# kofinandi/pixel-nerf-yolo

Measured on AMD Instinct MI355X. Metric: rays/sec (whole node), 64 samples/ray, 3-view 128×128 render, higher is better.
Workload: dtype f32 (matrix products on f16x2 split operands, fp32 accumulate)

## Files before the change

pixel-nerf-yolo_amd/csrc/mlp_h2.hip:

```cpp
#include <cstdlib>
#include <cstring>
#include <cstdio>
#include <vector>

#include "mlp_bwd_core.h"
#include "mlp_h2_core.h"

#if PNY_H2_PLANES == 1
#define PNY_H2_KERNEL pny_mlp_h1_kernel
#elif defined(PNY_H2_SPLIT)
#define PNY_H2_KERNEL pny_mlp_h2s_kernel
#else
#define PNY_H2_KERNEL pny_mlp_h2_kernel
#endif

namespace pny {

#ifdef PNY_H2_STAMP
enum { HS_TOTAL = 0, HS_GEMM, HS_GATHER_WAIT, HS_GATHER, HS_EPI_WAIT, HS_EPI, HS_PROLOGUE, HS_LINOUT, HS_SLAB, HS_REAL, HS_N };
__device__ unsigned long long* g_h2_stamp_buf;
__device__ __forceinline__ unsigned long long h2now() {
    unsigned long long t;
    __builtin_amdgcn_sched_barrier(0);
    asm volatile("s_memtime %0\n\ts_waitcnt lgkmcnt(0)" : "=s"(t)::"memory");
    __builtin_amdgcn_sched_barrier(0);
    return t;
}
#define HS_T0() hs_t_ = h2now()
#define HS_LAP(cat)                         \
    {                                       \
        const unsigned long long n_ = h2now(); \
        hs_acc[cat] += n_ - hs_t_;          \
        hs_t_ = n_;                         \
    }
#else
#define HS_T0()
#define HS_LAP(cat)
#endif


__device__ __forceinline__ void stash_store(__amdgpu_buffer_rsrc_t rsrc, unsigned voff, unsigned soff, float a, float b, float c, float d) {
    const f32x4 v = {a, b, c, d};
    __builtin_amdgcn_raw_buffer_store_b128(__builtin_bit_cast(u32x4, v), rsrc, voff + soff, 0, 0);
}

template <bool SIGNED = false>
__device__ __forceinline__ void h2put_planes(char* slot, float r0, float r1, float r2, float r3, float& rmax) {
    if constexpr (SIGNED)
        rmax = fmaxf(fmaxf(rmax, fmaxf(fabsf(r0), fabsf(r1))), fmaxf(fabsf(r2), fabsf(r3)));
    else
        rmax = fmaxf(fmaxf(rmax, fmaxf(r0, r1)), fmaxf(r2, r3));
    put_planes(slot, r0, r1, r2, r3);
}
__device__ __forceinline__ void range_check(float rmax, unsigned* range_flag) {
    if (__builtin_expect(!(rmax < 65520.0f), 0)) range_report(range_flag, 1u);
}

template <bool ADDZ, bool STASH = false>
__device__ __forceinline__ void h2epilogue(f32x16 (&acc)[h2::NT][h2::MT], const float* bias, char* planes, int wave, int lane, unsigned* range_flag,
                                           __amdgpu_buffer_rsrc_t stash = __amdgpu_buffer_rsrc_t(), unsigned stash_off = 0) {
    using namespace h2;
    const unsigned stash_lane = (unsigned)(((8 * NT * wave + (lane >> 5)) * TM + (lane & 31)) * 16);
    const int m0 = lane & 31, hh = lane >> 5;
    const float* bl = bias + 32 * NT * wave + 4 * hh;
    float rmax = 0.f;
    char* base = planes + (4 * NT * wave) * (2 * ROW_BYTES) + m0 * 16 + 8 * hh;
#pragma unroll
    for (int nt = 0; nt < NT; ++nt) {
        float4 b[4];
#pragma unroll
        for (int q = 0; q < 4; ++q) b[q] = *reinterpret_cast<const float4*>(bl + 32 * nt + 8 * q);
#pragma unroll
        for (int mt = 0; mt < MT; ++mt) {
            float2 za[4], zb[4];
            if (ADDZ) {
#pragma unroll
                for (int q = 0; q < 4; ++q) {
                    const char* s0 = base + (4 * nt + q) * (2 * ROW_BYTES) + 32 * mt * 16;
                    za[q] = *reinterpret_cast<const float2*>(s0);
                    zb[q] = *reinterpret_cast<const float2*>(s0 + ROW_BYTES);
                }
            }
            __builtin_amdgcn_sched_barrier(0);
#pragma unroll
            for (int q = 0; q < 4; ++q) {
                char* s0 = base + (4 * nt + q) * (2 * ROW_BYTES) + 32 * mt * 16;
                float x0 = acc[nt][mt][4 * q + 0] + b[q].x, x1 = acc[nt][mt][4 * q + 1] + b[q].y;
                float x2 = acc[nt][mt][4 * q + 2] + b[q].z, x3 = acc[nt][mt][4 * q + 3] + b[q].w;
                if (ADDZ) {
                    x0 += za[q].x;
                    x1 += za[q].y;
                    x2 += zb[q].x;
                    x3 += zb[q].y;
                }
                acc[nt][mt][4 * q + 0] = x0;
                acc[nt][mt][4 * q + 1] = x1;
                acc[nt][mt][4 * q + 2] = x2;
                acc[nt][mt][4 * q + 3] = x3;
                const float r0 = relu1(x0), r1 = relu1(x1), r2 = relu1(x2), r3 = relu1(x3);
                if constexpr (STASH) stash_store(stash, stash_lane, stash_off + (unsigned)(((8 * nt + 2 * q) * TM + 32 * mt) * 16), r0, r1, r2, r3);
                h2put_planes(s0, r0, r1, r2, r3, rmax);
            }
        }
    }
    range_check(rmax, range_flag);
}

struct SlabRef {
    __amdgpu_buffer_rsrc_t rsrc;
    unsigned lane_off;
};
__device__ __forceinline__ void h2slab_store(const f32x16 (&h)[h2::NT][h2::MT], const SlabRef& sl) {
    using namespace h2;
#pragma unroll
    for (int nt = 0; nt < NT; ++nt)
#pragma unroll
        for (int mt = 0; mt < MT; ++mt)
#pragma unroll
            for (int q = 0; q < 4; ++q) {
// ... 4 lines not shown
}
__device__ __forceinline__ void h2slab_load(f32x16 (&t)[h2::NT][h2::MT], const SlabRef& sl) {
    using namespace h2;
#pragma unroll
    for (int nt = 0; nt < NT; ++nt)
#pragma unroll
        for (int mt = 0; mt < MT; ++mt)
#pragma unroll
            for (int q = 0; q < 4; ++q) {
                const u32x4 u = __builtin_amdgcn_raw_buffer_load_b128(sl.rsrc, sl.lane_off, (unsigned)(((nt * MT + mt) * 4 + q) * 64 * 16), 2);
                const f32x4 v = __builtin_bit_cast(f32x4, u);
                t[nt][mt][4 * q + 0] = v.x;
                t[nt][mt][4 * q + 1] = v.y;
                t[nt][mt][4 * q + 2] = v.z;
                t[nt][mt][4 * q + 3] = v.w;
            }
}

#ifndef PNY_H2_SLAB_DEPTH
#define PNY_H2_SLAB_DEPTH 4
#endif
struct SlabPipe {
    static constexpr int SD = PNY_H2_SLAB_DEPTH;
    static_assert(SD >= 2, "slab pipeline");
    f32x4 buf[SD][4];
};
__device__ __forceinline__ void h2slab_issue(SlabPipe& sp, int p, const SlabRef& sh, const SlabRef& sr) {
    const SlabRef& s = (p & 1) ? sh : sr;
#pragma unroll
    for (int q = 0; q < 4; ++q)
        sp.buf[p % SlabPipe::SD][q] =
            __builtin_bit_cast(f32x4, __builtin_amdgcn_raw_buffer_load_b128(s.rsrc, s.lane_off, (unsigned)(((p >> 1) * 4 + q) * 64 * 16), 2));
}
__device__ __forceinline__ void h2view_sum(f32x16 (&net)[h2::NT][h2::MT], f32x16 (&h)[h2::NT][h2::MT], const float* bias, const SlabRef& sh,
                                           const SlabRef& sr, bool add, bool store, int wave, int lane) {
    using namespace h2;
    SlabPipe sp;
    const float* bl = bias + 32 * NT * wave + 4 * (lane >> 5);
    constexpr int NP = 2 * NT * MT, SD = SlabPipe::SD;
    if (add) {
#pragma unroll
        for (int p = 0; p + 1 < SD; ++p) h2slab_issue(sp, p, sh, sr);
    }
#pragma unroll
    for (int p = 0; p < NP; ++p) {
        const int nt = (p >> 1) / MT, mt = (p >> 1) % MT;
        if (add) {
            if (p + SD - 1 < NP) h2slab_issue(sp, p + SD - 1, sh, sr);
            __builtin_amdgcn_sched_barrier(0);
        }
        f32x16& t = (p & 1) ? h[nt][mt] : net[nt][mt];
#pragma unroll
        for (int q = 0; q < 4; ++q) {
            if (!(p & 1)) {
                const float4 b = *reinterpret_cast<const float4*>(bl + 32 * nt + 8 * q);
                t[4 * q + 0] = relu1(t[4 * q + 0] + b.x);
                t[4 * q + 1] = relu1(t[4 * q + 1] + b.y);
                t[4 * q + 2] = relu1(t[4 * q + 2] + b.z);
                t[4 * q + 3] = relu1(t[4 * q + 3] + b.w);
            }
            if (add) {
#pragma unroll
                for (int i = 0; i < 4; ++i) t[4 * q + i] = t[4 * q + i] + sp.buf[p % SD][q][i];
            }
            if (store) {
                const SlabRef& s = (p & 1) ? sh : sr;
                const f32x4 v = {t[4 * q + 0], t[4 * q + 1], t[4 * q + 2], t[4 * q + 3]};
                __builtin_amdgcn_raw_buffer_store_b128(__builtin_bit_cast(u32x4, v), s.rsrc, s.lane_off + (unsigned)(((p >> 1) * 4 + q) * 64 * 16), 0, 2);
            }
        }
        if (add) __builtin_amdgcn_sched_barrier(0);
    }
}

__device__ __forceinline__ void h2mean_planes(const f32x16 (&net)[h2::NT][h2::MT], f32x16 (&h)[h2::NT][h2::MT], float rns, char* planes, int wave,
                                              int lane, unsigned* range_flag) {
    using namespace h2;
    float rmax = 0.f;
    char* base = planes + (4 * NT * wave) * (2 * ROW_BYTES) + (lane & 31) * 16 + 8 * (lane >> 5);
#pragma unroll
    for (int nt = 0; nt < NT; ++nt)
#pragma unroll
        for (int mt = 0; mt < MT; ++mt)
#pragma unroll
            for (int q = 0; q < 4; ++q) {
                char* s0 = base + (4 * nt + q) * (2 * ROW_BYTES) + 32 * mt * 16;
                const float r0 = net[nt][mt][4 * q + 0] * rns, r1 = net[nt][mt][4 * q + 1] * rns;
                const float r2 = net[nt][mt][4 * q + 2] * rns, r3 = net[nt][mt][4 * q + 3] * rns;
                h2put_planes(s0, r0, r1, r2, r3, rmax);
#pragma unroll
                for (int i = 0; i < 4; ++i) h[nt][mt][4 * q + i] = h[nt][mt][4 * q + i] * rns;
            }
    range_check(rmax, range_flag);
}

template <int B>
__device__ __forceinline__ void h2gather_commit(const GatherTaps<h2::C, 2>& g, char* planes, int chunk, int wave, int lane) {
    using namespace h2;
    constexpr int NMB = GatherTaps<C>::NMB, QSTEP = GatherTaps<C>::QSTEP;
    const int m = (wave % NMB) * 8 + (lane & 7);
    char* base = planes + (16 * chunk + (lane >> 4)) * (2 * ROW_BYTES) + m * 16 + 8 * ((lane >> 3) & 1);
#pragma unroll
    for (int i = 0; i < GatherTaps<C>::QPW; ++i) {
        const int qb = wave / NMB + i * QSTEP;
        const float4 r = tap_blend(g.x[B][i], g.w);
        char* s0 = base + (4 * qb) * (2 * ROW_BYTES);
        *reinterpret_cast<float2*>(s0) = make_float2(r.x, r.y);
        *reinterpret_cast<float2*>(s0 + ROW_BYTES) = make_float2(r.z, r.w);
    }
}

struct WaveGather {
    f32x4 x[2][4][4];
};
template <int B, int T>
__device__ __forceinline__ void h2wave_issue(WaveGather& wg, __amdgpu_buffer_rsrc_t zr, const float4* tap_tab, unsigned c0, int lane) {
    using namespace h2;
    constexpr int nt = T / MT, mt = T % MT;
    asm volatile("" : "+v"(lane));
    const float4* tt = tap_tab + 2 * (32 * mt + (lane >> 3));
    const unsigned ql = 16u * (unsigned)(lane & 7);
#pragma unroll
    for (int pass = 0; pass < 4; ++pass) {
        const float4 o = tt[16 * pass];
        const unsigned off[4] = {(unsigned)__float_as_int(o.x), (unsigned)__float_as_int(o.y), (unsigned)__float_as_int(o.z), (unsigned)__float_as_int(o.w)};
#pragma unroll
        for (int k = 0; k < 4; ++k)
            wg.x[B][pass][k] = __builtin_bit_cast(f32x4, __builtin_amdgcn_raw_buffer_load_b128(zr, off[k] * 4u + ql, c0 + 128u * nt, 0));
    }
}
template <int B, int T>
__device__ __forceinline__ void h2wave_commit(const WaveGather& wg, f32x16 (&acc)[h2::NT][h2::MT], const float4* tap_tab, const float* bias,
                                              char* planes, int wave, int lane, float& rmax) {
    using namespace h2;
    constexpr int nt = T / MT, mt = T % MT;
    const int jq = lane & 7, sl = lane >> 3, m0 = lane & 31, hh = lane >> 5;
    char* tb = planes + (4 * NT * wave + 4 * nt) * (2 * ROW_BYTES) + 32 * mt * 16;
    char* wr = tb + jq * ROW_BYTES + 16 * (sl ^ jq);
    const float4* tw = tap_tab + 2 * (32 * mt + sl) + 1;
#pragma unroll
    for (int pass = 0; pass < 4; ++pass) {
        const float4 w4 = tw[16 * pass];
        const float w[4] = {w4.x, w4.y, w4.z, w4.w};
        float4 x[4];
#pragma unroll
        for (int k = 0; k < 4; ++k) x[k] = make_float4(wg.x[B][pass][k][0], wg.x[B][pass][k][1], wg.x[B][pass][k][2], wg.x[B][pass][k][3]);
        *reinterpret_cast<float4*>(wr + 128 * pass) = tap_blend(x, w);
    }
    __builtin_amdgcn_fence(__ATOMIC_RELEASE, "wavefront");
    __builtin_amdgcn_wave_barrier();
    __builtin_amdgcn_fence(__ATOMIC_ACQUIRE, "wavefront");
    const float* bl = bias + 32 * NT * wave + 32 * nt + 4 * hh;
    auto rd_b = [&](int q) { return *reinterpret_cast<const float4*>(bl + 8 * q); };
    auto rd_z = [&](int q) { return *reinterpret_cast<const float4*>(tb + (2 * q + hh) * ROW_BYTES + 16 * (m0 ^ (2 * q + hh))); };
    float4 b = rd_b(0), z = rd_z(0);
#pragma unroll
    for (int q = 0; q < 4; ++q) {
        const float4 bq = b, zq = z;
        if (q + 1 < 4) b = rd_b(q + 1), z = rd_z(q + 1);
        __builtin_amdgcn_fence(__ATOMIC_ACQ_REL, "wavefront");
        char* s0 = tb + q * (2 * ROW_BYTES) + m0 * 16 + 8 * hh;
        float x0 = acc[nt][mt][4 * q + 0] + bq.x, x1 = acc[nt][mt][4 * q + 1] + bq.y;
        float x2 = acc[nt][mt][4 * q + 2] + bq.z, x3 = acc[nt][mt][4 * q + 3] + bq.w;
        x0 += zq.x;
        x1 += zq.y;
        x2 += zq.z;
        x3 += zq.w;
        acc[nt][mt][4 * q + 0] = x0;
        acc[nt][mt][4 * q + 1] = x1;
        acc[nt][mt][4 * q + 2] = x2;
        acc[nt][mt][4 * q + 3] = x3;
        const float r0 = relu1(x0), r1 = relu1(x1), r2 = relu1(x2), r3 = relu1(x3);
        h2put_planes(s0, r0, r1, r2, r3, rmax);
    }
}
__device__ __forceinline__ void h2wave_entry(WaveGather& wg, f32x16 (&acc)[h2::NT][h2::MT], __amdgpu_buffer_rsrc_t zr, const float4* tap_tab, unsigned c0,
                                             const float* bias, char* planes, int wave, int lane, unsigned* range_flag) {
    static_assert(h2::NT * h2::MT == 4, "four sub-chunks");
    asm volatile("" : "+v"(lane));
    float rmax = 0.f;
    h2wave_issue<1, 1>(wg, zr, tap_tab, c0, lane);
    __builtin_amdgcn_sched_barrier(0);
    h2wave_commit<0, 0>(wg, acc, tap_tab, bias, planes, wave, lane, rmax);
    h2wave_issue<0, 2>(wg, zr, tap_tab, c0, lane);
    __builtin_amdgcn_sched_barrier(0);
    h2wave_commit<1, 1>(wg, acc, tap_tab, bias, planes, wave, lane, rmax);
    h2wave_issue<1, 3>(wg, zr, tap_tab, c0, lane);
    __builtin_amdgcn_sched_barrier(0);
    h2wave_commit<0, 2>(wg, acc, tap_tab, bias, planes, wave, lane, rmax);
    h2wave_commit<1, 3>(wg, acc, tap_tab, bias, planes, wave, lane, rmax);
    range_check(rmax, range_flag);
}

#if PNY_H2_PLANES == 2
struct LinOutW {
    h8 f[2 * h2::NT][2];
};
__device__ __forceinline__ void h2linout_issue(LinOutW& lw, const WStream& ws, unsigned img_off, int nto_n, int nto, int wave) {
    using namespace h2;
    unsigned base = img_off + (unsigned)(((2 * NT * wave * nto_n + nto) * 2) * 64) * 16u, step = (unsigned)(nto_n * 2 * 64) * 16u;
    asm volatile("" : "+s"(base), "+s"(step));
#pragma unroll
    for (int ks = 0; ks < 2 * NT; ++ks)
#pragma unroll
        for (int p = 0; p < 2; ++p)
            lw.f[ks][p] = __builtin_bit_cast(h8, __builtin_amdgcn_raw_buffer_load_b128(ws.rsrc, ws.lane_off, base + ks * step + (unsigned)(p * 64) * 16u, 0));
}
constexpr int LINOUT_WAVE_BYTES = 4 * h2::NT * 2 * h2::ROW_BYTES;
static_assert((h2::NT / 2) * h2::TM * 16 * 16 <= LINOUT_WAVE_BYTES, "a wave's partials (64 outputs) fit its own rows");
__device__ __forceinline__ void h2linout_product(LinOutW& lw, const WStream& ws, unsigned img_off, int d_out, char* planes, int wave, int lane) {
    using namespace h2;
    constexpr int NCH = NT / 2;
    asm volatile("" : "+v"(lane));
    const int m0 = lane & 31, hh = lane >> 5;
    const int qo = (d_out + 3) >> 2, nto_n = d_out > 32 ? 2 : 1;
    char* region = planes + wave * LINOUT_WAVE_BYTES;
    __builtin_amdgcn_fence(__ATOMIC_RELEASE, "wavefront");
    __builtin_amdgcn_wave_barrier();
    __builtin_amdgcn_fence(__ATOMIC_ACQUIRE, "wavefront");
    h8 B[NCH][MT][4][2];
#pragma unroll
    for (int c = 0; c < NCH; ++c)
#pragma unroll
// ... 42 lines not shown
    static_assert(NCHUNK * 64 == HID, "eight chunks of 64 k");
    asm volatile("" : "+v"(tid));
    const int qo = (a.d_out + 3) >> 2;
    const bool vec = a.d_out == 4 && (reinterpret_cast<size_t>(a.out) & 15) == 0;
    for (int idx = tid; idx < qo * TM; idx += THREADS) {
        const int qd = idx / TM, m = idx % TM;
        const char* src = planes + (m * qo + qd) * 16;
        f32x4 part[NCHUNK];
#pragma unroll
        for (int g = 0; g < NCHUNK; ++g) part[g] = *reinterpret_cast<const f32x4*>(src + (g / NCH) * LINOUT_WAVE_BYTES + (g % NCH) * (TM * qo * 16));
        float sum[4];
#pragma unroll
        for (int i = 0; i < 4; ++i) {
            sum[i] = part[0][i];
#pragma unroll
            for (int g = 1; g < NCHUNK; ++g) sum[i] = sum[i] + part[g][i];
        }
        const long long s = tile * TM + m;
        if (s >= a.n_points) continue;
        if (vec) {
#pragma unroll
            for (int i = 0; i < 4; ++i) sum[i] = output_head(sum[i] + a.w.b_out[i], i, a.yolo);
            *reinterpret_cast<float4*>(a.out + s * 4) = make_float4(sum[0], sum[1], sum[2], sum[3]);
        } else {
#pragma unroll
            for (int i = 0; i < 4; ++i) {
                const int o = 4 * qd + i;
                if (o < a.d_out) a.out[s * a.d_out + o] = output_head(sum[i] + a.w.b_out[o], o, a.yolo);
            }
        }
    }
}
#endif

template <bool STASH>
__device__ __forceinline__ void h2prologue(const MlpArgs& a, int v, long long tile, char* planes, float4* tap_tab, int tid, unsigned* range_flag,
                                           __amdgpu_buffer_rsrc_t stash = __amdgpu_buffer_rsrc_t(), unsigned stash_xin = 0, float4* tap_raw = nullptr) {
    using namespace h2;
    constexpr int NPART = THREADS / TM;
    const int m = tid % TM, part = tid / TM;
    long long s = tile * TM + m;
    if (s >= a.n_points) s = a.n_points - 1;
    float p[3], d[3];
    load_point(a, s, p, d);
    const Cam cam = a.cams[tile_view_base(a, tile * TM) + v];
    float xr[3], xc[3], vd[3];
    camera_point(cam, p, d, xr, xc, vd);
    float rmax = 0.f;
    for (int g = part; g < D_IN_PAD / 4; g += NPART) {
        const float e0 = input_entry(4 * g + 0, xr, vd, a.freq_factor, a.num_freqs), e1 = input_entry(4 * g + 1, xr, vd, a.freq_factor, a.num_freqs);
        const float e2 = input_entry(4 * g + 2, xr, vd, a.freq_factor, a.num_freqs), e3 = input_entry(4 * g + 3, xr, vd, a.freq_factor, a.num_freqs);
        if constexpr (STASH) stash_store(stash, (unsigned)((g * TM + m) * 16), stash_xin, e0, e1, e2, e3);
        h2put_planes<true>(planes + (g >> 1) * (2 * ROW_BYTES) + m * 16 + 8 * (g & 1), e0, e1, e2, e3, rmax);
    }
    range_check(rmax, range_flag);
    if (part == NPART - 1) {
        int pix[4], offs[4];
        float wgt[4];
        pixel_taps(a, cam, xc, 1, pix, wgt);
#pragma unroll
        for (int k = 0; k < 4; ++k) offs[k] = pix[k] * a.tap_stride;
        tap_record(tap_tab, m, offs, wgt);
        if constexpr (STASH) {
#pragma unroll
            for (int k = 0; k < 4; ++k) offs[k] = pix[k] * a.L;
            tap_record(tap_raw, m, offs, wgt);
        }
    }
}

template <bool STASH>
__global__ __launch_bounds__(h2::THREADS, 2) void PNY_H2_KERNEL(const MlpArgs a) {
    using namespace h2;
    extern __shared__ __attribute__((aligned(16))) char smem_raw[];
    char* planes = smem_raw;
    float4* tap_tab = reinterpret_cast<float4*>(smem_raw + ACT_BYTES);
    float* bias_tab = reinterpret_cast<float*>(smem_raw + ACT_BYTES + TAP_BYTES);
    float4* tap_raw = reinterpret_cast<float4*>(smem_raw + lds_bytes(a.n_blocks));
    const int tid = threadIdx.x, lane = tid & 63, wave = __builtin_amdgcn_readfirstlane(tid >> 6);
    const SlabRef slab = {__builtin_amdgcn_make_buffer_rsrc(a.scratch + (size_t)blockIdx.x * (TM * HID), 0, TM * HID * 4, 0x00020000),
                          (unsigned)((wave * (NT * MT * 16 * 64) + 4 * lane) * 4)};
#if defined(PNY_H2_PER_VIEW_FC1) || PNY_H2_PLANES == 1
    constexpr bool VIEW_MEAN = false;
#else
    constexpr bool VIEW_MEAN = !STASH;
#endif
    constexpr bool WAVE_ENTRY = !STASH;
    const SlabRef slab_r = {__builtin_amdgcn_make_buffer_rsrc(a.scratch + ((size_t)gridDim.x + blockIdx.x) * (TM * HID), 0, TM * HID * 4, 0x00020000),
                            slab.lane_off};
    const int nb = a.n_blocks;
    const int nvb = a.combine_layer < nb ? a.combine_layer : nb;
    const WStream ws = wstream(a, lane);
    const H2Seg s_in = h2seg(ws, a.h2_in, D_IN_PAD / 16, wave);
    auto fc0seg = [&](int b) { return h2seg(ws, a.h2_fc0[b], HID / 16, wave); };
    auto fc1seg = [&](int b) { return h2seg(ws, a.h2_fc1[b], HID / 16, wave); };
    auto entry_bias = [&](int b) -> const float* {
        if constexpr (LDS_BIAS) return bias_tab + (b == 0 ? 0 : 2 * b) * HID;
        return b == 0 ? a.w.b_in : a.w.b_fc1[b - 1];
    };
    auto fc0_bias = [&](int b) -> const float* {
        if constexpr (LDS_BIAS) return bias_tab + (1 + 2 * b) * HID;
        return a.w.b_fc0[b];
    };
    H2Ring ring;
    h2ring_fill(ring, ws, s_in);
#ifdef PNY_H2_STAMP
    unsigned long long hs_acc[HS_N], hs_t_ = 0;
    for (int i = 0; i < HS_N; ++i) hs_acc[i] = 0;
    const unsigned long long hs_start = h2now();
    const unsigned long long hs_real0 = __builtin_amdgcn_s_memrealtime();
#endif
    if constexpr (LDS_BIAS) {
        for (int i = tid; i < (1 + 2 * nb) * HID; i += THREADS) {
            const int vec = i / HID, f = i % HID;
            const float* src = vec == 0 ? a.w.b_in : ((vec & 1) ? a.w.b_fc0[(vec - 1) >> 1] : a.w.b_fc1[(vec - 2) >> 1]);
            bias_tab[i] = src[f];
        }
    }

    const TileWalk tw = tile_walk(a.n_tiles);
    for (long long tile = tw.first; tile < tw.last; tile += tw.step) {
        f32x16 h[NT][MT];
        f32x16 net[NT][MT];
        GatherTaps<C, 2> g;
        WaveGather wg;
        __amdgpu_buffer_rsrc_t zr = __amdgpu_buffer_rsrc_t();
        const unsigned wave_c0 = (unsigned)(32 * NT * wave) * 4u;
        auto prefetch = [&](int c0) {
            if constexpr (WAVE_ENTRY)
                h2wave_issue<0, 0>(wg, zr, tap_tab, (unsigned)c0 * 4u + wave_c0, lane);
            else
                gather_issue<C, 0>(g, c0, wave);
        };
        __amdgpu_buffer_rsrc_t xr = __amdgpu_buffer_rsrc_t();
        if constexpr (STASH)
            xr = stash_rsrc(a.lay.x_record(a.stash_x, tile), a.lay.x_tile);
        auto block_tail = [&](int blk, const H2Seg& after, bool slab_in, int next_c0, unsigned stash_net) {
            HS_T0();
            h2zero<NT, MT>(net);
            __syncthreads();
            HS_LAP(HS_EPI_WAIT);
            h2gemm(net, ring, ws, fc0seg(blk), fc1seg(blk), planes, lane);
            HS_LAP(HS_GEMM);
            __syncthreads();
            HS_LAP(HS_EPI_WAIT);
            h2epilogue<false, STASH>(net, fc0_bias(blk), planes, wave, lane, a.range_flag, xr, stash_net);
            if (!VIEW_MEAN && slab_in) {
                h2slab_load(net, slab);
                HS_LAP(HS_EPI);
                __syncthreads();
                HS_LAP(HS_EPI_WAIT);
                h2gemm(h, ring, ws, fc1seg(blk), after, planes, lane);
                HS_LAP(HS_GEMM);
#pragma unroll
                for (int nt = 0; nt < NT; ++nt)
#pragma unroll
                    for (int mt = 0; mt < MT; ++mt)
#pragma unroll
                        for (int r = 0; r < 16; ++r) h[nt][mt][r] = net[nt][mt][r] + h[nt][mt][r];
            } else if (next_c0 >= 0) {
                HS_LAP(HS_EPI);
                __syncthreads();
                HS_LAP(HS_EPI_WAIT);
                h2gemm(h, ring, ws, fc1seg(blk), after, planes, lane, [&]() { prefetch(next_c0); });
                HS_LAP(HS_GEMM);
            } else {
                HS_LAP(HS_EPI);
                __syncthreads();
                HS_LAP(HS_EPI_WAIT);
                h2gemm(h, ring, ws, fc1seg(blk), after, planes, lane);
                HS_LAP(HS_GEMM);
            }
        };
        for (int v = 0; v < a.NS; ++v) {
            const int vb = tile_view_base(a, tile * TM);
            const H2Seg after_view = v + 1 < a.NS ? s_in : (nvb < nb ? fc0seg(nvb) : s_in);
            const unsigned x_view = STASH ? stash_bytes((unsigned)v * (unsigned)a.lay.x_view) : 0u;
            auto act_slot = [&](int i) { return x_view + stash_bytes((unsigned)a.lay.o_act + (unsigned)i * (unsigned)STASH_SLOT); };
            HS_T0();
            __syncthreads();
            h2prologue<STASH>(a, v, tile, planes, tap_tab, tid, a.range_flag, xr, x_view + stash_bytes((unsigned)a.lay.o_in), tap_raw);
            h2zero<NT, MT>(h);
            __syncthreads();
            if constexpr (STASH) {
                const unsigned xz = x_view + stash_bytes((unsigned)a.lay.o_z);
                gather_setup<C>(g, a.latent + (size_t)(vb + v) * a.Hl * a.Wl * a.L, tap_raw, wave, lane);
                const int nch = a.L / GCH;
                const unsigned zlane = (unsigned)(((lane >> 3) * TM + (wave % 8) * 8 + (lane & 7)) * 16);
                auto put = [&](const float4(&x)[4][4], int c) {
#pragma unroll
                    for (int i = 0; i < 4; ++i) {
                        const float4 r = tap_blend(x[i], g.w);
                        stash_store(xr, zlane, xz + (unsigned)((32 * c + 8 * i) * TM * 16), r.x, r.y, r.z, r.w);
                    }
                };
                gather_issue<C, 0>(g, 0, wave);
                for (int c = 0; c < nch; c += 2) {
                    if (c + 1 < nch) gather_issue<C, 1>(g, (c + 1) * GCH, wave);
                    __builtin_amdgcn_sched_barrier(0);
                    put(g.x[0], c);
                    if (c + 2 < nch) gather_issue<C, 0>(g, (c + 2) * GCH, wave);
                    __builtin_amdgcn_sched_barrier(0);
                    if (c + 1 < nch) put(g.x[1], c + 1);
                }
            }
            if constexpr (WAVE_ENTRY) {
                const size_t zfloats = (size_t)a.Hl * a.Wl * a.zp_stride;
                zr = __builtin_amdgcn_make_buffer_rsrc(const_cast<float*>(a.zp) + (size_t)(vb + v) * zfloats, 0, (int)(unsigned)(zfloats * 4), 0x00020000);
            } else {
                gather_setup<C>(g, a.zp + (size_t)(vb + v) * a.Hl * a.Wl * a.zp_stride, tap_tab, wave, lane);
            }
            prefetch(0);
            HS_LAP(HS_PROLOGUE);
            h2gemm(h, ring, ws, s_in, fc0seg(0), planes, lane);
            HS_LAP(HS_GEMM);
            auto block_entry = [&](int blk) {
                const int cb = blk * HID;
                HS_LAP(HS_GATHER);
                __syncthreads();
                HS_LAP(HS_GATHER_WAIT);
                if constexpr (WAVE_ENTRY) {
                    h2wave_entry(wg, h, zr, tap_tab, (unsigned)cb * 4u + wave_c0, entry_bias(blk), planes, wave, lane, a.range_flag);
                    HS_LAP(HS_GATHER);
                    return;
                }
                gather_issue<C, 1>(g, cb + GCH, wave);
                __builtin_amdgcn_sched_barrier(0);
                h2gather_commit<0>(g, planes, 0, wave, lane);
                gather_issue<C, 0>(g, cb + 2 * GCH, wave);
                __builtin_amdgcn_sched_barrier(0);
                h2gather_commit<1>(g, planes, 1, wave, lane);
                gather_issue<C, 1>(g, cb + 3 * GCH, wave);
                __builtin_amdgcn_sched_barrier(0);
                h2gather_commit<0>(g, planes, 2, wave, lane);
                h2gather_commit<1>(g, planes, 3, wave, lane);
                HS_LAP(HS_GATHER);
                __syncthreads();
                HS_LAP(HS_GATHER_WAIT);
                h2epilogue<true, STASH>(h, entry_bias(blk), planes, wave, lane, a.range_flag, xr, act_slot(2 * blk));
                HS_LAP(HS_EPI);
            };
            auto view_block = [&](int blk, const H2Seg& after, bool slab_in, int next_c0) {
                block_entry(blk);
                block_tail(blk, after, slab_in, next_c0, act_slot(2 * blk + 1));
            };
            auto mean_tail = [&](int blk) {
                const bool last = v + 1 == a.NS;
                HS_T0();
                h2zero<NT, MT>(net);
                __syncthreads();
                HS_LAP(HS_EPI_WAIT);
                h2gemm(net, ring, ws, fc0seg(blk), last ? fc1seg(blk) : s_in, planes, lane);
                HS_LAP(HS_GEMM);
                h2view_sum(net, h, fc0_bias(blk), slab, slab_r, v > 0, !last, wave, lane);
                if (!last) {
                    HS_LAP(HS_SLAB);
                    return;
                }
                HS_LAP(v > 0 ? HS_SLAB : HS_EPI);
                __syncthreads();
                HS_LAP(HS_EPI_WAIT);
                h2mean_planes(net, h, 1.0f / (float)a.NS, planes, wave, lane, a.range_flag);
                HS_LAP(HS_EPI);
                __syncthreads();
                HS_LAP(HS_EPI_WAIT);
                h2gemm(h, ring, ws, fc1seg(blk), after_view, planes, lane);
                HS_LAP(HS_GEMM);
            };
#if defined(PNY_H2_NOPREFETCH)
            for (int blk = 0; blk + 1 < nvb; ++blk) {
                view_block(blk, fc0seg(blk + 1), false, -1);
                prefetch((blk + 1) * HID);
            }
#else
            for (int blk = 0; blk + 1 < nvb; ++blk) view_block(blk, fc0seg(blk + 1), false, (blk + 1) * HID);
#endif
            if constexpr (VIEW_MEAN) {
                block_entry(nvb - 1);
                mean_tail(nvb - 1);
            } else {
                view_block(nvb - 1, after_view, v > 0, -1);
            }
            if (!VIEW_MEAN && a.NS > 1) {
                HS_T0();
                if (v + 1 < a.NS) {
                    h2slab_store(h, slab);
                } else {
                    const float rns = 1.0f / (float)a.NS;
#pragma unroll
                    for (int nt = 0; nt < NT; ++nt)
#pragma unroll
                        for (int mt = 0; mt < MT; ++mt)
#pragma unroll
                            for (int r = 0; r < 16; ++r) h[nt][mt][r] = h[nt][mt][r] * rns;
                }
                HS_LAP(HS_SLAB);
            }
        }
        auto post_slot = [&](int i) { return stash_bytes((unsigned)a.lay.x_post + (unsigned)i * (unsigned)STASH_SLOT); };
        for (int blk = nvb; blk < nb; ++blk) {
            HS_T0();
            __syncthreads();
            HS_LAP(HS_EPI_WAIT);
            h2epilogue<false, STASH>(h, entry_bias(blk), planes, wave, lane, a.range_flag, xr, post_slot(2 * (blk - nvb)));
            HS_LAP(HS_EPI);
            block_tail(blk, blk + 1 < nb ? fc0seg(blk + 1) : s_in, false, -1, post_slot(2 * (blk - nvb) + 1));
        }
        HS_T0();
#if PNY_H2_PLANES == 2
        const unsigned out_off = (unsigned)(reinterpret_cast<const char*>(a.h2_out) - ws.base);
        LinOutW lw;
        h2linout_issue(lw, ws, out_off, a.d_out > 32 ? 2 : 1, 0, wave);
        __builtin_amdgcn_sched_barrier(0);
        __syncthreads();
        h2epilogue<false, STASH>(h, entry_bias(nb), planes, wave, lane, a.range_flag, xr, post_slot(2 * (nb - nvb)));
        h2linout_product(lw, ws, out_off, a.d_out, planes, wave, lane);
        __syncthreads();
        h2linout_reduce(a, tile, planes, tid);
#else
        __syncthreads();
        h2epilogue<false, STASH>(h, entry_bias(nb), planes, wave, lane, a.range_flag, xr, post_slot(2 * (nb - nvb)));
        __syncthreads();
        for (int idx = tid; idx < a.d_out * TM; idx += THREADS) {
            const int o = idx / TM, m = idx % TM;
            const float4* wrow = reinterpret_cast<const float4*>(a.w.w_out + (size_t)o * HID);
            float sum = 0.f;
#pragma unroll 4
            for (int kg = 0; kg < HID / 8; ++kg) {
                const h8 x0 = *reinterpret_cast<const h8*>(planes + kg * (2 * ROW_BYTES) + m * 16);
                const float4 wa = wrow[2 * kg], wb = wrow[2 * kg + 1];
                sum += (float)x0[0] * wa.x;
                sum += (float)x0[1] * wa.y;
                sum += (float)x0[2] * wa.z;
                sum += (float)x0[3] * wa.w;
                sum += (float)x0[4] * wb.x;
                sum += (float)x0[5] * wb.y;
                sum += (float)x0[6] * wb.z;
                sum += (float)x0[7] * wb.w;
            }
            sum = output_head(sum + a.w.b_out[o], o, a.yolo);
            const long long s = tile * TM + m;
            if (s < a.n_points) a.out[s * a.d_out + o] = sum;
        }
#endif
        HS_LAP(HS_LINOUT);
    }
#ifdef PNY_H2_STAMP
    hs_acc[HS_TOTAL] = h2now() - hs_start;
    hs_acc[HS_REAL] = __builtin_amdgcn_s_memrealtime() - hs_real0;
    if (lane == 0)
        for (int i = 0; i < HS_N; ++i) g_h2_stamp_buf[((size_t)blockIdx.x * (THREADS / 64) + wave) * HS_N + i] = hs_acc[i];
#endif
}

// ... 49 lines not shown
```

pixel-nerf-yolo_amd/csrc/mlp_h2_core.h:

```cpp
#pragma once
#include "mlp_core.h"

namespace pny {

typedef _Float16 h8 __attribute__((ext_vector_type(8)));
typedef _Float16 h4 __attribute__((ext_vector_type(4)));

namespace h2 {
#ifndef PNY_H2_PLANES
#define PNY_H2_PLANES 2
#endif
#ifndef PNY_H2_WD
#if PNY_H2_PLANES == 1
#define PNY_H2_WD 4
#else
#define PNY_H2_WD 2
#endif
#endif
#ifndef PNY_H2_NT
#define PNY_H2_NT 2
#endif
#ifndef PNY_H2_MT
#define PNY_H2_MT 2
#endif
// ... 154 lines not shown
#pragma unroll
            for (int i = 0; i < NT * MT; ++i) {
                __builtin_amdgcn_sched_group_barrier(0x008, 1, 0);
                if (i < 2) __builtin_amdgcn_sched_group_barrier(0x100, 1, 0);
                __builtin_amdgcn_sched_group_barrier(0x006, 2, 0);
            }
#endif
            __builtin_amdgcn_sched_barrier(0);
            if constexpr (MT > 1) {
#pragma unroll
                for (int p = 0; p < 2; ++p) B[(d + 1) & 1][MT - 1][p] = *reinterpret_cast<const h8*>(bj + p * ROW_BYTES + 32 * 16);
            }
#pragma unroll
            for (int nt = 0; nt < NT; ++nt)
#pragma unroll
                for (int mt = 0; mt < MT; ++mt)
                    acc[nt][mt] = h2mfma(r.f[d][nt][1], B[d & 1][mt][0], acc[nt][mt]);
#ifndef PNY_H2_NOSCHED
#pragma unroll
            for (int i = 0; i < NT * MT; ++i) {
                __builtin_amdgcn_sched_group_barrier(0x008, 1, 0);
                if (MT > 1 && i < 2) __builtin_amdgcn_sched_group_barrier(0x100, 1, 0);
                __builtin_amdgcn_sched_group_barrier(0x006, 2, 0);
            }
#endif
#pragma unroll
            for (int mt = 0; mt < MT; ++mt)
#pragma unroll
                for (int p = 0; p < 2; ++p) asm volatile("" ::"v"(B[d & 1][mt][p]));
        }
    }
#endif
}

__device__ __forceinline__ void split2(float a, float b, unsigned& p0, unsigned& p1) {
#ifdef PNY_H2_PLAIN_SPLIT
    typedef _Float16 h2v __attribute__((ext_vector_type(2)));
    h2v q0, q1;
    q0[0] = (_Float16)a;
    q0[1] = (_Float16)b;
    q1[0] = (_Float16)(a - (float)q0[0]);
    q1[1] = (_Float16)(b - (float)q0[1]);
    p0 = __builtin_bit_cast(unsigned, q0);
    p1 = __builtin_bit_cast(unsigned, q1);
#else
    float ra, rb;
    asm("v_cvt_pk_f16_f32 %0, %1, %2" : "=v"(p0) : "v"(a), "v"(b));
    asm("v_fma_mix_f32 %0, %1, -1.0, %2 op_sel_hi:[1,0,0]" : "=v"(ra) : "v"(p0), "v"(a));
    asm("v_fma_mix_f32 %0, %1, -1.0, %2 op_sel:[1,0,0] op_sel_hi:[1,0,0]" : "=v"(rb) : "v"(p0), "v"(b));
    asm("v_cvt_pk_f16_f32 %0, %1, %2" : "=v"(p1) : "v"(ra), "v"(rb));
#endif
}
__device__ __forceinline__ void split4(float a, float b, float c, float d, h4& p0, h4& p1) {
    uint2 u0, u1;
    split2(a, b, u0.x, u1.x);
    split2(c, d, u0.y, u1.y);
    p0 = __builtin_bit_cast(h4, u0);
    p1 = __builtin_bit_cast(h4, u1);
}

__device__ __forceinline__ h4 cvt4(float a, float b, float c, float d) {
    uint2 u;
    asm("v_cvt_pk_f16_f32 %0, %1, %2" : "=v"(u.x) : "v"(a), "v"(b));
    asm("v_cvt_pk_f16_f32 %0, %1, %2" : "=v"(u.y) : "v"(c), "v"(d));
    return __builtin_bit_cast(h4, u);
}
// ... 24 lines not shown
```

Baseline: 230,800.

## Use 16x16x32 f16 MFMA tiles for the non-stash two-plane MLP GEMM path

```diff
diff --git a/pixel-nerf-yolo_amd/csrc/mlp_h2.hip b/pixel-nerf-yolo_amd/csrc/mlp_h2.hip
--- a/pixel-nerf-yolo_amd/csrc/mlp_h2.hip
+++ b/pixel-nerf-yolo_amd/csrc/mlp_h2.hip
@@ -56,27 +56,28 @@
     if (__builtin_expect(!(rmax < 65520.0f), 0)) range_report(range_flag, 1u);
 }
 
-template <bool ADDZ, bool STASH = false>
+template <bool ADDZ, bool STASH = false, bool M16 = false>
 __device__ __forceinline__ void h2epilogue(f32x16 (&acc)[h2::NT][h2::MT], const float* bias, char* planes, int wave, int lane, unsigned* range_flag,
                                            __amdgpu_buffer_rsrc_t stash = __amdgpu_buffer_rsrc_t(), unsigned stash_off = 0) {
     using namespace h2;
+    static_assert(!M16 || (!ADDZ && !STASH), "the shared entry and the stash are laid out for the 32 x 32 accumulator tile");
+    using Q = H2Quad<M16>;
     const unsigned stash_lane = (unsigned)(((8 * NT * wave + (lane >> 5)) * TM + (lane & 31)) * 16);
-    const int m0 = lane & 31, hh = lane >> 5;
-    const float* bl = bias + 32 * NT * wave + 4 * hh;
+    const float* bl = bias + 32 * NT * wave + Q::lane_feat(lane);
     float rmax = 0.f;
-    char* base = planes + (4 * NT * wave) * (2 * ROW_BYTES) + m0 * 16 + 8 * hh;
+    char* base = Q::slot_lane(planes + (4 * NT * wave) * (2 * ROW_BYTES), lane);
 #pragma unroll
     for (int nt = 0; nt < NT; ++nt) {
         float4 b[4];
 #pragma unroll
-        for (int q = 0; q < 4; ++q) b[q] = *reinterpret_cast<const float4*>(bl + 32 * nt + 8 * q);
+        for (int q = 0; q < 4; ++q) b[q] = *reinterpret_cast<const float4*>(bl + Q::feat(nt, q));
 #pragma unroll
         for (int mt = 0; mt < MT; ++mt) {
             float2 za[4], zb[4];
             if (ADDZ) {
 #pragma unroll
                 for (int q = 0; q < 4; ++q) {
-                    const char* s0 = base + (4 * nt + q) * (2 * ROW_BYTES) + 32 * mt * 16;
+                    const char* s0 = base + Q::slot_off(nt, mt, q);
                     za[q] = *reinterpret_cast<const float2*>(s0);
                     zb[q] = *reinterpret_cast<const float2*>(s0 + ROW_BYTES);
                 }
@@ -84,7 +85,7 @@
             __builtin_amdgcn_sched_barrier(0);
 #pragma unroll
             for (int q = 0; q < 4; ++q) {
-                char* s0 = base + (4 * nt + q) * (2 * ROW_BYTES) + 32 * mt * 16;
+                char* s0 = base + Q::slot_off(nt, mt, q);
                 float x0 = acc[nt][mt][4 * q + 0] + b[q].x, x1 = acc[nt][mt][4 * q + 1] + b[q].y;
                 float x2 = acc[nt][mt][4 * q + 2] + b[q].z, x3 = acc[nt][mt][4 * q + 3] + b[q].w;
                 if (ADDZ) {
@@ -155,11 +156,15 @@
         sp.buf[p % SlabPipe::SD][q] =
             __builtin_bit_cast(f32x4, __builtin_amdgcn_raw_buffer_load_b128(s.rsrc, s.lane_off, (unsigned)(((p >> 1) * 4 + q) * 64 * 16), 2));
 }
+template <bool M16>
 __device__ __forceinline__ void h2view_sum(f32x16 (&net)[h2::NT][h2::MT], f32x16 (&h)[h2::NT][h2::MT], const float* bias, const SlabRef& sh,
                                            const SlabRef& sr, bool add, bool store, int wave, int lane) {
     using namespace h2;
+    using Q = H2Quad<M16>;
     SlabPipe sp;
-    const float* bl = bias + 32 * NT * wave + 4 * (lane >> 5);
+    unsigned slab_lane = sh.lane_off;
+    asm volatile("" : "+v"(slab_lane));
+    const float* bl = bias + 32 * NT * wave + Q::lane_feat(lane);
     constexpr int NP = 2 * NT * MT, SD = SlabPipe::SD;
     if (add) {
 #pragma unroll
@@ -176,7 +181,7 @@
 #pragma unroll
         for (int q = 0; q < 4; ++q) {
             if (!(p & 1)) {
-                const float4 b = *reinterpret_cast<const float4*>(bl + 32 * nt + 8 * q);
+                const float4 b = *reinterpret_cast<const float4*>(bl + Q::feat(nt, q));
                 t[4 * q + 0] = relu1(t[4 * q + 0] + b.x);
                 t[4 * q + 1] = relu1(t[4 * q + 1] + b.y);
                 t[4 * q + 2] = relu1(t[4 * q + 2] + b.z);
@@ -189,25 +194,26 @@
             if (store) {
                 const SlabRef& s = (p & 1) ? sh : sr;
                 const f32x4 v = {t[4 * q + 0], t[4 * q + 1], t[4 * q + 2], t[4 * q + 3]};
-                __builtin_amdgcn_raw_buffer_store_b128(__builtin_bit_cast(u32x4, v), s.rsrc, s.lane_off + (unsigned)(((p >> 1) * 4 + q) * 64 * 16), 0, 2);
+                __builtin_amdgcn_raw_buffer_store_b128(__builtin_bit_cast(u32x4, v), s.rsrc, slab_lane + (unsigned)(((p >> 1) * 4 + q) * 64 * 16), 0, 2);
             }
         }
         if (add) __builtin_amdgcn_sched_barrier(0);
     }
 }
 
+template <bool M16>
 __device__ __forceinline__ void h2mean_planes(const f32x16 (&net)[h2::NT][h2::MT], f32x16 (&h)[h2::NT][h2::MT], float rns, char* planes, int wave,
                                               int lane, unsigned* range_flag) {
     using namespace h2;
     float rmax = 0.f;
-    char* base = planes + (4 * NT * wave) * (2 * ROW_BYTES) + (lane & 31) * 16 + 8 * (lane >> 5);
+    char* base = H2Quad<M16>::slot_lane(planes + (4 * NT * wave) * (2 * ROW_BYTES), lane);
 #pragma unroll
     for (int nt = 0; nt < NT; ++nt)
 #pragma unroll
         for (int mt = 0; mt < MT; ++mt)
 #pragma unroll
             for (int q = 0; q < 4; ++q) {
-                char* s0 = base + (4 * nt + q) * (2 * ROW_BYTES) + 32 * mt * 16;
+                char* s0 = base + H2Quad<M16>::slot_off(nt, mt, q);
                 const float r0 = net[nt][mt][4 * q + 0] * rns, r1 = net[nt][mt][4 * q + 1] * rns;
                 const float r2 = net[nt][mt][4 * q + 2] * rns, r3 = net[nt][mt][4 * q + 3] * rns;
                 h2put_planes(s0, r0, r1, r2, r3, rmax);
@@ -252,12 +258,14 @@
             wg.x[B][pass][k] = __builtin_bit_cast(f32x4, __builtin_amdgcn_raw_buffer_load_b128(zr, off[k] * 4u + ql, c0 + 128u * nt, 0));
     }
 }
-template <int B, int T>
+template <int B, int T, bool M16>
 __device__ __forceinline__ void h2wave_commit(const WaveGather& wg, f32x16 (&acc)[h2::NT][h2::MT], const float4* tap_tab, const float* bias,
                                               char* planes, int wave, int lane, float& rmax) {
     using namespace h2;
     constexpr int nt = T / MT, mt = T % MT;
-    const int jq = lane & 7, sl = lane >> 3, m0 = lane & 31, hh = lane >> 5;
+    using Q = H2Quad<M16>;
+    const int jq = lane & 7, sl = lane >> 3;
+    const int zj = Q::lane_feat(lane) >> 2, zs = Q::lane_samp(lane);
     char* tb = planes + (4 * NT * wave + 4 * nt) * (2 * ROW_BYTES) + 32 * mt * 16;
     char* wr = tb + jq * ROW_BYTES + 16 * (sl ^ jq);
     const float4* tw = tap_tab + 2 * (32 * mt + sl) + 1;
@@ -273,16 +281,19 @@
     __builtin_amdgcn_fence(__ATOMIC_RELEASE, "wavefront");
     __builtin_amdgcn_wave_barrier();
     __builtin_amdgcn_fence(__ATOMIC_ACQUIRE, "wavefront");
-    const float* bl = bias + 32 * NT * wave + 32 * nt + 4 * hh;
-    auto rd_b = [&](int q) { return *reinterpret_cast<const float4*>(bl + 8 * q); };
-    auto rd_z = [&](int q) { return *reinterpret_cast<const float4*>(tb + (2 * q + hh) * ROW_BYTES + 16 * (m0 ^ (2 * q + hh))); };
+    const float* bl = bias + 32 * NT * wave + 32 * nt + Q::lane_feat(lane);
+    auto rd_b = [&](int q) { return *reinterpret_cast<const float4*>(bl + Q::feat(0, q)); };
+    auto rd_z = [&](int q) {
+        const int j = (Q::feat(0, q) >> 2) + zj, s = Q::samp(0, q) + zs;
+        return *reinterpret_cast<const float4*>(tb + j * ROW_BYTES + 16 * (s ^ j));
+    };
     float4 b = rd_b(0), z = rd_z(0);
 #pragma unroll
     for (int q = 0; q < 4; ++q) {
         const float4 bq = b, zq = z;
         if (q + 1 < 4) b = rd_b(q + 1), z = rd_z(q + 1);
         __builtin_amdgcn_fence(__ATOMIC_ACQ_REL, "wavefront");
-        char* s0 = tb + q * (2 * ROW_BYTES) + m0 * 16 + 8 * hh;
+        char* s0 = Q::slot_lane(tb + Q::slot_off(0, 0, q), lane);
         float x0 = acc[nt][mt][4 * q + 0] + bq.x, x1 = acc[nt][mt][4 * q + 1] + bq.y;
         float x2 = acc[nt][mt][4 * q + 2] + bq.z, x3 = acc[nt][mt][4 * q + 3] + bq.w;
         x0 += zq.x;
@@ -297,6 +308,7 @@
         h2put_planes(s0, r0, r1, r2, r3, rmax);
     }
 }
+template <bool M16>
 __device__ __forceinline__ void h2wave_entry(WaveGather& wg, f32x16 (&acc)[h2::NT][h2::MT], __amdgpu_buffer_rsrc_t zr, const float4* tap_tab, unsigned c0,
                                              const float* bias, char* planes, int wave, int lane, unsigned* range_flag) {
     static_assert(h2::NT * h2::MT == 4, "four sub-chunks");
@@ -304,14 +316,14 @@
     float rmax = 0.f;
     h2wave_issue<1, 1>(wg, zr, tap_tab, c0, lane);
     __builtin_amdgcn_sched_barrier(0);
-    h2wave_commit<0, 0>(wg, acc, tap_tab, bias, planes, wave, lane, rmax);
+    h2wave_commit<0, 0, M16>(wg, acc, tap_tab, bias, planes, wave, lane, rmax);
     h2wave_issue<0, 2>(wg, zr, tap_tab, c0, lane);
     __builtin_amdgcn_sched_barrier(0);
-    h2wave_commit<1, 1>(wg, acc, tap_tab, bias, planes, wave, lane, rmax);
+    h2wave_commit<1, 1, M16>(wg, acc, tap_tab, bias, planes, wave, lane, rmax);
     h2wave_issue<1, 3>(wg, zr, tap_tab, c0, lane);
     __builtin_amdgcn_sched_barrier(0);
-    h2wave_commit<0, 2>(wg, acc, tap_tab, bias, planes, wave, lane, rmax);
-    h2wave_commit<1, 3>(wg, acc, tap_tab, bias, planes, wave, lane, rmax);
+    h2wave_commit<0, 2, M16>(wg, acc, tap_tab, bias, planes, wave, lane, rmax);
+    h2wave_commit<1, 3, M16>(wg, acc, tap_tab, bias, planes, wave, lane, rmax);
     range_check(rmax, range_flag);
 }
 
@@ -420,6 +432,17 @@
     }
 }
 #endif
+
+template <bool M16, class Side = NoSide>
+__device__ __forceinline__ void h2gemm_on(f32x16 (&acc)[h2::NT][h2::MT], H2Ring& r, const WStream& ws, const H2Seg& cur, const H2Seg& next,
+                                          const char* planes, int lane, Side side = Side()) {
+#if PNY_H2_PLANES == 2
+    if constexpr (M16)
+        h2gemm16(acc, r, ws, cur, next, planes, lane, side);
+    else
+#endif
+        h2gemm(acc, r, ws, cur, next, planes, lane, side);
+}
 
 template <bool STASH>
 __device__ __forceinline__ void h2prologue(const MlpArgs& a, int v, long long tile, char* planes, float4* tap_tab, int tid, unsigned* range_flag,
@@ -474,6 +497,7 @@
     constexpr bool VIEW_MEAN = !STASH;
 #endif
     constexpr bool WAVE_ENTRY = !STASH;
+    constexpr bool M16 = !STASH && PL == 2;
     const SlabRef slab_r = {__builtin_amdgcn_make_buffer_rsrc(a.scratch + ((size_t)gridDim.x + blockIdx.x) * (TM * HID), 0, TM * HID * 4, 0x00020000),
                             slab.lane_off};
     const int nb = a.n_blocks;
@@ -491,7 +515,12 @@
         return a.w.b_fc0[b];
     };
     H2Ring ring;
-    h2ring_fill(ring, ws, s_in);
+#if PNY_H2_PLANES == 2
+    if constexpr (M16)
+        h2ring_fill16(ring, ws, s_in, lane);
+    else
+#endif
+        h2ring_fill(ring, ws, s_in);
 #ifdef PNY_H2_STAMP
     unsigned long long hs_acc[HS_N], hs_t_ = 0;
     for (int i = 0; i < HS_N; ++i) hs_acc[i] = 0;
@@ -528,17 +557,17 @@
             h2zero<NT, MT>(net);
             __syncthreads();
             HS_LAP(HS_EPI_WAIT);
-            h2gemm(net, ring, ws, fc0seg(blk), fc1seg(blk), planes, lane);
+            h2gemm_on<M16>(net, ring, ws, fc0seg(blk), fc1seg(blk), planes, lane);
             HS_LAP(HS_GEMM);
             __syncthreads();
             HS_LAP(HS_EPI_WAIT);
-            h2epilogue<false, STASH>(net, fc0_bias(blk), planes, wave, lane, a.range_flag, xr, stash_net);
+            h2epilogue<false, STASH, M16>(net, fc0_bias(blk), planes, wave, lane, a.range_flag, xr, stash_net);
             if (!VIEW_MEAN && slab_in) {
                 h2slab_load(net, slab);
                 HS_LAP(HS_EPI);
                 __syncthreads();
                 HS_LAP(HS_EPI_WAIT);
-                h2gemm(h, ring, ws, fc1seg(blk), after, planes, lane);
+                h2gemm_on<M16>(h, ring, ws, fc1seg(blk), after, planes, lane);
                 HS_LAP(HS_GEMM);
 #pragma unroll
                 for (int nt = 0; nt < NT; ++nt)
@@ -550,13 +579,19 @@
                 HS_LAP(HS_EPI);
                 __syncthreads();
                 HS_LAP(HS_EPI_WAIT);
-                h2gemm(h, ring, ws, fc1seg(blk), after, planes, lane, [&]() { prefetch(next_c0); });
+                if constexpr (M16) {
+#pragma unroll
+                    for (int pass = 0; pass < 4; ++pass)
+#pragma unroll
+                        for (int k = 0; k < 4; ++k) wg.x[0][pass][k] = __builtin_nondeterministic_value(wg.x[0][pass][k]);
+                }
+                h2gemm_on<M16>(h, ring, ws, fc1seg(blk), after, planes, lane, [&]() { prefetch(next_c0); });
                 HS_LAP(HS_GEMM);
             } else {
                 HS_LAP(HS_EPI);
                 __syncthreads();
                 HS_LAP(HS_EPI_WAIT);
-                h2gemm(h, ring, ws, fc1seg(blk), after, planes, lane);
+                h2gemm_on<M16>(h, ring, ws, fc1seg(blk), after, planes, lane);
                 HS_LAP(HS_GEMM);
             }
         };
@@ -600,7 +635,7 @@
             }
             prefetch(0);
             HS_LAP(HS_PROLOGUE);
-            h2gemm(h, ring, ws, s_in, fc0seg(0), planes, lane);
+            h2gemm_on<M16>(h, ring, ws, s_in, fc0seg(0), planes, lane);
             HS_LAP(HS_GEMM);
             auto block_entry = [&](int blk) {
                 const int cb = blk * HID;
@@ -608,7 +643,7 @@
                 __syncthreads();
                 HS_LAP(HS_GATHER_WAIT);
                 if constexpr (WAVE_ENTRY) {
-                    h2wave_entry(wg, h, zr, tap_tab, (unsigned)cb * 4u + wave_c0, entry_bias(blk), planes, wave, lane, a.range_flag);
+                    h2wave_entry<M16>(wg, h, zr, tap_tab, (unsigned)cb * 4u + wave_c0, entry_bias(blk), planes, wave, lane, a.range_flag);
                     HS_LAP(HS_GATHER);
                     return;
                 }
@@ -638,9 +673,9 @@
                 h2zero<NT, MT>(net);
                 __syncthreads();
                 HS_LAP(HS_EPI_WAIT);
-                h2gemm(net, ring, ws, fc0seg(blk), last ? fc1seg(blk) : s_in, planes, lane);
+                h2gemm_on<M16>(net, ring, ws, fc0seg(blk), last ? fc1seg(blk) : s_in, planes, lane);
                 HS_LAP(HS_GEMM);
-                h2view_sum(net, h, fc0_bias(blk), slab, slab_r, v > 0, !last, wave, lane);
+                h2view_sum<M16>(net, h, fc0_bias(blk), slab, slab_r, v > 0, !last, wave, lane);
                 if (!last) {
                     HS_LAP(HS_SLAB);
                     return;
@@ -648,11 +683,11 @@
                 HS_LAP(v > 0 ? HS_SLAB : HS_EPI);
                 __syncthreads();
                 HS_LAP(HS_EPI_WAIT);
-                h2mean_planes(net, h, 1.0f / (float)a.NS, planes, wave, lane, a.range_flag);
+                h2mean_planes<M16>(net, h, 1.0f / (float)a.NS, planes, wave, lane, a.range_flag);
                 HS_LAP(HS_EPI);
                 __syncthreads();
                 HS_LAP(HS_EPI_WAIT);
-                h2gemm(h, ring, ws, fc1seg(blk), after_view, planes, lane);
+                h2gemm_on<M16>(h, ring, ws, fc1seg(blk), after_view, planes, lane);
                 HS_LAP(HS_GEMM);
             };
 #if defined(PNY_H2_NOPREFETCH)
@@ -690,7 +725,7 @@
             HS_T0();
             __syncthreads();
             HS_LAP(HS_EPI_WAIT);
-            h2epilogue<false, STASH>(h, entry_bias(blk), planes, wave, lane, a.range_flag, xr, post_slot(2 * (blk - nvb)));
+            h2epilogue<false, STASH, M16>(h, entry_bias(blk), planes, wave, lane, a.range_flag, xr, post_slot(2 * (blk - nvb)));
             HS_LAP(HS_EPI);
             block_tail(blk, blk + 1 < nb ? fc0seg(blk + 1) : s_in, false, -1, post_slot(2 * (blk - nvb) + 1));
         }
@@ -701,13 +736,13 @@
         h2linout_issue(lw, ws, out_off, a.d_out > 32 ? 2 : 1, 0, wave);
         __builtin_amdgcn_sched_barrier(0);
         __syncthreads();
-        h2epilogue<false, STASH>(h, entry_bias(nb), planes, wave, lane, a.range_flag, xr, post_slot(2 * (nb - nvb)));
+        h2epilogue<false, STASH, M16>(h, entry_bias(nb), planes, wave, lane, a.range_flag, xr, post_slot(2 * (nb - nvb)));
         h2linout_product(lw, ws, out_off, a.d_out, planes, wave, lane);
         __syncthreads();
         h2linout_reduce(a, tile, planes, tid);
 #else
         __syncthreads();
-        h2epilogue<false, STASH>(h, entry_bias(nb), planes, wave, lane, a.range_flag, xr, post_slot(2 * (nb - nvb)));
+        h2epilogue<false, STASH, M16>(h, entry_bias(nb), planes, wave, lane, a.range_flag, xr, post_slot(2 * (nb - nvb)));
         __syncthreads();
         for (int idx = tid; idx < a.d_out * TM; idx += THREADS) {
             const int o = idx / TM, m = idx % TM;
diff --git a/pixel-nerf-yolo_amd/csrc/mlp_h2_core.h b/pixel-nerf-yolo_amd/csrc/mlp_h2_core.h
--- a/pixel-nerf-yolo_amd/csrc/mlp_h2_core.h
+++ b/pixel-nerf-yolo_amd/csrc/mlp_h2_core.h
@@ -210,6 +210,118 @@
     }
 #endif
 }
+
+#if PNY_H2_PLANES == 2 && PNY_H2_WD == 2
+__device__ __forceinline__ f32x4 h2mfma16(h8 a, h8 b, f32x4 c) { return __builtin_amdgcn_mfma_f32_16x16x32_f16(a, b, c, 0, 0, 0); }
+constexpr unsigned H2_STEP_BYTES = 16u * h2::PL * 64u * 16u;
+__device__ __forceinline__ unsigned h2sub_off(unsigned seg_off, int j, int nt, int nlo, int p) {
+    return seg_off + (unsigned)j * (2u * H2_STEP_BYTES) + (unsigned)((nt * 2 + p) * 64 + 16 * nlo) * 16u;
+}
+__device__ __forceinline__ h8 h2load16(const WStream& ws, unsigned lane_off, unsigned sub_off) {
+    return __builtin_bit_cast(h8, __builtin_amdgcn_raw_buffer_load_b128(ws.rsrc, lane_off, sub_off, PNY_H2_WAUX));
+}
+__device__ __forceinline__ unsigned h2lane_off16(int lane) {
+    return (unsigned)(lane >> 5) * H2_STEP_BYTES + (unsigned)((lane & 15) + 32 * ((lane >> 4) & 1)) * 16u;
+}
+__device__ __forceinline__ void h2ring_fill16(H2Ring& r, const WStream& ws, const H2Seg& s, int lane) {
+    static_assert(h2::WD == 2 && h2::PL == 2 && h2::NT % 2 == 0, "one ring slot per sub-step, two slots");
+    const unsigned wl = h2lane_off16(lane);
+#pragma unroll
+    for (int nlo = 0; nlo < 2; ++nlo)
+#pragma unroll
+        for (int p = 0; p < 2; ++p) {
+            r.f[0][nlo][p] = h2load16(ws, wl, h2sub_off(s.off, 0, 0, nlo, p));
+            r.f[1][nlo][p] = h8{0, 0, 0, 0, 0, 0, 0, 0};
+        }
+}
+template <class Side = NoSide>
+__device__ __forceinline__ void h2gemm16(f32x16 (&acc)[h2::NT][h2::MT], H2Ring& r, const WStream& ws, const H2Seg& cur, const H2Seg& next,
+                                         const char* planes, int lane, Side side = Side()) {
+    using namespace h2;
+    constexpr int M4 = 2 * MT;
+    const unsigned wl = h2lane_off16(lane);
+    const char* bp = planes + (lane >> 4) * (2 * ROW_BYTES) + (lane & 15) * 16;
+    const int jn = cur.jn >> 1, jl = jn - 1;
+    h8 B[M4][2];
+#pragma unroll
+    for (int m4 = 0; m4 < M4; ++m4)
+#pragma unroll
+        for (int p = 0; p < 2; ++p) B[m4][p] = *reinterpret_cast<const h8*>(bp + p * ROW_BYTES + 16 * m4 * 16);
+    for (int j = 0; j < jn; ++j) {
+        if (j == 1) side();
+        const char* bj = bp + ((j < jl) ? j + 1 : jl) * (8 * ROW_BYTES);
+        const bool in_cur = j < jl;
+#pragma unroll
+        for (int nt = 0; nt < NT; ++nt) {
+            const int d = nt & 1;
+            const unsigned src = (nt + 1 < NT || in_cur) ? cur.off : next.off;
+            const int jx = nt + 1 < NT ? j : (in_cur ? j + 1 : 0);
+            unsigned so[2][2];
+#pragma unroll
+            for (int nlo = 0; nlo < 2; ++nlo)
+#pragma unroll
+                for (int p = 0; p < 2; ++p) {
+                    so[nlo][p] = h2sub_off(src, jx, (nt + 1) % NT, nlo, p);
+                    asm volatile("" : "+s"(so[nlo][p]));
+                }
+            __builtin_amdgcn_sched_barrier(0);
+#pragma unroll
+            for (int nlo = 0; nlo < 2; ++nlo)
+#pragma unroll
+                for (int p = 0; p < 2; ++p) r.f[d ^ 1][nlo][p] = h2load16(ws, wl, so[nlo][p]);
+#pragma unroll
+            for (int m4 = 0; m4 < M4; ++m4) {
+                const int mt = m4 >> 1, mlo = m4 & 1;
+                if (nt == NT - 1 && m4 > 0) {
+#pragma unroll
+                    for (int p = 0; p < 2; ++p) B[m4 - 1][p] = *reinterpret_cast<const h8*>(bj + p * ROW_BYTES + 16 * (m4 - 1) * 16);
+                }
+#pragma unroll
+                for (int t = 0; t < 3; ++t)
+#pragma unroll
+                    for (int nlo = 0; nlo < 2; ++nlo) {
+                        const int q = 2 * nlo + mlo;
+                        f32x16& A = acc[nt][mt];
+                        const f32x4 c = {A[4 * q + 0], A[4 * q + 1], A[4 * q + 2], A[4 * q + 3]};
+                        const f32x4 o = h2mfma16(r.f[d][nlo][t == 2], B[m4][t == 1], c);
+                        A[4 * q + 0] = o[0];
+                        A[4 * q + 1] = o[1];
+                        A[4 * q + 2] = o[2];
+                        A[4 * q + 3] = o[3];
+                    }
+#ifndef PNY_H2_NOSCHED
+#pragma unroll
+                for (int i = 0; i < 6; ++i) {
+                    __builtin_amdgcn_sched_group_barrier(0x008, 1, 0);
+                    if (nt == NT - 1 && m4 > 0 && i < 2) __builtin_amdgcn_sched_group_barrier(0x100, 1, 0);
+                    if (m4 == 0 && i < 4) __builtin_amdgcn_sched_group_barrier(0x020, 1, 0);
+                    __builtin_amdgcn_sched_group_barrier(0x006, 2, 0);
+                }
+#endif
+                __builtin_amdgcn_sched_barrier(0);
+            }
+            if (nt == NT - 1) {
+#pragma unroll
+                for (int p = 0; p < 2; ++p) B[M4 - 1][p] = *reinterpret_cast<const h8*>(bj + p * ROW_BYTES + 16 * (M4 - 1) * 16);
+            }
+        }
+    }
+}
+
+#endif
+
+template <bool M16>
+struct H2Quad {
+    __device__ static __forceinline__ int lane_feat(int lane) { return 4 * (lane >> (M16 ? 4 : 5)); }
+    __device__ static __forceinline__ int lane_samp(int lane) { return lane & (M16 ? 15 : 31); }
+    __device__ static constexpr int feat(int nt, int q) { return 32 * nt + (M16 ? 16 * (q >> 1) : 8 * q); }
+    __device__ static constexpr int samp(int mt, int q) { return 32 * mt + (M16 ? 16 * (q & 1) : 0); }
+    __device__ static __forceinline__ char* slot_lane(char* rows, int lane) {
+        if constexpr (!M16) return rows + (lane & 31) * 16 + 8 * (lane >> 5);
+        return rows + (lane & 15) * 16 + 8 * ((lane >> 4) & 1) + (lane >> 5) * (2 * h2::ROW_BYTES);
+    }
+    __device__ static constexpr int slot_off(int nt, int mt, int q) { return (feat(nt, q) >> 3) * (2 * h2::ROW_BYTES) + samp(mt, q) * 16; }
+};
 
 __device__ __forceinline__ void split2(float a, float b, unsigned& p0, unsigned& p1) {
 #ifdef PNY_H2_PLAIN_SPLIT
```

Result: no change. 235,100 (median of 3 runs) (+1.8%).
